# nextpyp/spr_pick

Measured on AMD Instinct MI355X. Metric: train_patches_per_sec, higher is better.
Workload: dtype f32; 1 GPU; BASELINE configs[1]: ssdn --noise_style gaussian --noise_value var, joint mode, 64x64 patches from 4 synthetic 1024x1024 micrographs, batch 32 per GPU, alpha 0.75, tau 0.01, Adam; fp32 MFMA convolutions (Winograd F(2x2,3x3) for the wide 3x3 layers); per_gpu_batch=32, global_batch=32, patch=64, parallelism=single GPU

## Files before the change

include/sprk.h:

```cpp
#ifndef SPRK_H
#define SPRK_H

#include <stddef.h>
#include <stdint.h>

#ifdef __cplusplus
extern "C" {
#endif

#define SPRK_OK 0
#define SPRK_EINVAL (-1)
#define SPRK_EWORKSPACE (-2)
#define SPRK_ELAUNCH (-3)

#define SPRK_ACT_NONE 0
#define SPRK_ACT_LEAKY 1
#define SPRK_ACT_RELU 2

typedef struct sprk_conv_geom {
    int32_t N, C1, C2, Hin, Win, up1;
    int32_t Cout, Hout, Wout;
    int32_t KH, KW, stride, dil, pad_top, pad_left;
    int32_t dtype;
} sprk_conv_geom;
// ... 107 lines not shown
int sprk_act_bwd_partial(const void *gy, const void *y, void *gpre, float *gbias, int act,
                         int N, int C, int H, int W, int up2, long g_image_stride, int io,
                         void *ws, size_t ws_bytes, sprk_reduce_item *item, void *stream);
int sprk_reduce_items(const sprk_reduce_item *items, int n, void *stream);

int sprk_concat_up_bwd(const float *gin, float *ga, float *gb, int N, int C1, int C2, int H, int W,
                       int up1, void *stream);

int sprk_shift_maxpool2_fwd(const void *x, void *y, int NC, int H, int W, int shift, int io, void *stream);
int sprk_shift_maxpool2_bwd(const void *gy, const void *x, void *gx, int NC, int H, int W, int shift, int act,
                            int io, void *stream);
int sprk_rot4_stack_fwd(const float *x, float *y, int B, int C, int P, void *stream);
int sprk_rot4_stack_bwd(const float *gy, float *gx, int B, int C, int P, void *stream);
int sprk_unrot4_shift_concat_fwd(const void *d, void *f, int B, int C, int P, int io, void *stream);
int sprk_unrot4_shift_concat_bwd(const void *gf, void *gd, int B, int C, int P, int io, void *stream);
int sprk_unrot_act_bwd_eligible(int B, int C, int P, int act);
int sprk_conv2d_fwd_unrot_eligible(const sprk_conv_geom *g, const sprk_conv_epilogue *ep);
int sprk_conv2d_fwd_unrot(const float *x, const float *x2, const float *w, float *f, const sprk_conv_geom *g,
                          const sprk_conv_epilogue *ep, void *ws, size_t ws_bytes, void *stream);
int sprk_unrot_act_bwd(const float *gf, const float *f, float *gpre, float *gbias, int act, int B, int C, int P,
                       void *ws, size_t ws_bytes, sprk_reduce_item *item, void *stream);

size_t sprk_bn_ws_bytes(int N, int C, int HW, int groups);
int sprk_bn_train_fwd(const float *x, float *y, const float *gamma, const float *beta,
                      float *running_mean, float *running_var, float *save_mean, float *save_invstd,
                      int N, int C, int HW, int groups, float momentum, float eps, int relu,
                      void *ws, size_t ws_bytes, void *stream);
int sprk_bn_eval_fwd(const float *x, float *y, const float *gamma, const float *beta,
                     const float *running_mean, const float *running_var,
                     int N, int C, int HW, float eps, int relu, void *stream);
int sprk_bn_train_bwd(const float *gy, const float *x, const float *y, const float *gamma,
                      const float *save_mean, const float *save_invstd,
                      float *gx, float *ggamma, float *gbeta,
                      int N, int C, int HW, int groups, int relu, void *ws, size_t ws_bytes, void *stream);

int sprk_reparam_fwd(const float *out_stats, const float *eps, float *z, int B, int HW, void *stream);
int sprk_reparam_bwd(const float *gz, const float *out_stats, const float *eps, float *g_out_stats,
                     int B, int HW, void *stream);
int sprk_sigmoid_clamp_fwd(const float *x, float *p, long n, void *stream);
int sprk_sigmoid_clamp_bwd(const float *gp, const float *x, float *gx, long n, void *stream);
int sprk_crop_add_fwd(const float *y, const float *x, float *out, long NC, int Ho, int Wo, int Hx, int Wx, int off, int stride,
                      void *stream);
int sprk_crop_embed_bwd(const float *g, float *gx, long NC, int Ho, int Wo, int Hx, int Wx, int off, int stride, void *stream);
int sprk_noise_std_fwd(const float *est, float *noise_std, float *z, int B, int HW, void *stream);
int sprk_noise_std_bwd(const float *g, const float *z, float *g_est, int B, int HW, void *stream);
int sprk_joint_loss_fwd(const float *loss_out, const float *pred, const float *p, const float *pf, float *final_loss,
// ... 129 lines not shown
```

spr_pick_amd/_lib.py:

```python
import ctypes
import os

_HERE = os.path.dirname(os.path.abspath(__file__))
LIB_PATH = os.environ.get("SPRK_LIB") or os.path.join(_HERE, "libsprk.so")

ACT_NONE, ACT_LEAKY, ACT_RELU = 0, 1, 2
DT_F32, DT_BF16, DT_F16 = 0, 1, 2
DT_NAIVE = 0x200
DT_WPREP = 0x800
DT_X16, DT_Y16 = 0x8000, 0x10000
DT_PIN = 0x400
DT_FORCE = 0x100
DTYPES = {"f32": DT_F32, "fp32": DT_F32, "bf16": DT_BF16, "f16": DT_F16, "fp16": DT_F16,
          "bf16!": DT_BF16 | DT_FORCE, "f16!": DT_F16 | DT_FORCE}

c_f = ctypes.c_void_p
c_i = ctypes.c_int
c_vp = ctypes.c_void_p
c_sz = ctypes.c_size_t


class ConvGeom(ctypes.Structure):
    _fields_ = [(n, ctypes.c_int32) for n in
                ("N", "C1", "C2", "Hin", "Win", "up1", "Cout", "Hout", "Wout",
# ... 51 lines not shown
    "sprk_conv2d_storage16": (c_i, [ctypes.POINTER(ConvGeom), ctypes.POINTER(ConvEpilogue)]),
    "sprk_conv2d_bwd_weight": (c_i, [c_f, c_f, c_f, c_f, ctypes.POINTER(ConvGeom), c_vp, c_sz, c_vp]),
    "sprk_conv2d_bwd_weight_partial": (c_i, [c_f, c_f, c_f, c_f, ctypes.POINTER(ConvGeom), c_vp, c_sz, ctypes.POINTER(ReduceItem), c_vp]),
    "sprk_act_bwd_partial": (c_i, [c_f, c_f, c_f, c_f, c_i, c_i, c_i, c_i, c_i, c_i, ctypes.c_long, c_i, c_vp, c_sz, ctypes.POINTER(ReduceItem), c_vp]),
    "sprk_reduce_items": (c_i, [ctypes.POINTER(ReduceItem), c_i, c_vp]),
    "sprk_act_bwd_ws_bytes": (c_sz, [c_i, c_i, c_i]),
    "sprk_act_bwd": (c_i, [c_f, c_f, c_f, c_f, c_i, c_i, c_i, c_i, c_i, c_i, ctypes.c_long, c_i, c_vp, c_sz, c_vp]),
    "sprk_concat_up_bwd": (c_i, [c_f, c_f, c_f, c_i, c_i, c_i, c_i, c_i, c_i, c_vp]),
    "sprk_shift_maxpool2_fwd": (c_i, [c_f, c_f, c_i, c_i, c_i, c_i, c_i, c_vp]),
    "sprk_shift_maxpool2_bwd": (c_i, [c_f, c_f, c_f, c_i, c_i, c_i, c_i, c_i, c_i, c_vp]),
    "sprk_rot4_stack_fwd": (c_i, [c_f, c_f, c_i, c_i, c_i, c_vp]),
    "sprk_rot4_stack_bwd": (c_i, [c_f, c_f, c_i, c_i, c_i, c_vp]),
    "sprk_unrot4_shift_concat_fwd": (c_i, [c_f, c_f, c_i, c_i, c_i, c_i, c_vp]),
    "sprk_unrot4_shift_concat_bwd": (c_i, [c_f, c_f, c_i, c_i, c_i, c_i, c_vp]),
    "sprk_unrot_act_bwd_eligible": (c_i, [c_i, c_i, c_i, c_i]),
    "sprk_conv2d_fwd_unrot_eligible": (c_i, [ctypes.POINTER(ConvGeom), ctypes.POINTER(ConvEpilogue)]),
    "sprk_conv2d_bwd_data_mask_fused": (c_i, [ctypes.POINTER(ConvGeom)]),
    "sprk_conv2d_variant": (c_i, [c_i, ctypes.POINTER(ConvGeom), ctypes.POINTER(ConvEpilogue), c_vp, c_vp, c_vp,
                                  ctypes.POINTER(ctypes.c_int32)]),
    "sprk_conv2d_last_variant": (c_i, [c_i, ctypes.POINTER(ctypes.c_int32)]),
    "sprk_conv2d_fwd_unrot": (c_i, [c_f, c_f, c_f, c_f, ctypes.POINTER(ConvGeom), ctypes.POINTER(ConvEpilogue), c_vp, c_sz, c_vp]),
    "sprk_unrot_act_bwd": (c_i, [c_f, c_f, c_f, c_f, c_i, c_i, c_i, c_i, c_vp, c_sz, ctypes.POINTER(ReduceItem), c_vp]),
    "sprk_bn_ws_bytes": (c_sz, [c_i, c_i, c_i, c_i]),
    "sprk_bn_train_fwd": (c_i, [c_f, c_f, c_f, c_f, c_f, c_f, c_f, c_f, c_i, c_i, c_i, c_i, ctypes.c_float, ctypes.c_float, c_i, c_vp, c_sz, c_vp]),
    "sprk_bn_eval_fwd": (c_i, [c_f, c_f, c_f, c_f, c_f, c_f, c_i, c_i, c_i, ctypes.c_float, c_i, c_vp]),
    "sprk_bn_train_bwd": (c_i, [c_f, c_f, c_f, c_f, c_f, c_f, c_f, c_f, c_f, c_i, c_i, c_i, c_i, c_i, c_vp, c_sz, c_vp]),
    "sprk_crop_add_fwd": (c_i, [c_f, c_f, c_f, ctypes.c_long, c_i, c_i, c_i, c_i, c_i, c_i, c_vp]),
    "sprk_crop_embed_bwd": (c_i, [c_f, c_f, ctypes.c_long, c_i, c_i, c_i, c_i, c_i, c_i, c_vp]),
    "sprk_noise_std_fwd": (c_i, [c_f, c_f, c_f, c_i, c_i, c_vp]),
    "sprk_noise_std_bwd": (c_i, [c_f, c_f, c_f, c_i, c_i, c_vp]),
    "sprk_joint_loss_fwd": (c_i, [c_f, c_f, c_f, c_f, c_f, c_f, c_i, c_i, c_i, c_i, ctypes.c_float, ctypes.c_float, c_vp]),
    "sprk_joint_loss_bwd": (c_i, [c_f, c_f, c_f, c_f, c_f, c_f, c_f, c_i, c_i, c_i, c_i, ctypes.c_float, ctypes.c_float, c_vp]),
    "sprk_reparam_fwd": (c_i, [c_f, c_f, c_f, c_i, c_i, c_vp]),
    "sprk_reparam_bwd": (c_i, [c_f, c_f, c_f, c_f, c_i, c_i, c_vp]),
    "sprk_adam_multi": (c_i, [c_vp, c_vp, c_i, c_i, c_f, c_f, c_f, ctypes.c_float, ctypes.c_float, ctypes.c_float, c_vp]),
    "sprk_adam_multi_skip": (c_i, [c_vp, c_vp, c_i, c_i, c_f, c_f, c_f, ctypes.c_float, ctypes.c_float, ctypes.c_float, c_vp, c_vp]),
    "sprk_unscale_check": (c_i, [c_f, ctypes.c_long, c_f, c_vp, c_vp]),
    "sprk_loss_scale_update": (c_i, [c_f, c_f, c_vp, c_vp, c_vp, c_vp, ctypes.c_float, ctypes.c_float, c_i, c_vp]),
    "sprk_pu_loss": (c_i, [c_f, c_f, c_f, c_i, ctypes.c_float, c_f, c_f, c_vp]),
    "sprk_sigmoid_clamp_fwd": (c_i, [c_f, c_f, ctypes.c_long, c_vp]),
    "sprk_sigmoid_clamp_bwd": (c_i, [c_f, c_f, c_f, ctypes.c_long, c_vp]),
    "sprk_ssdn_ws_bytes": (c_sz, [c_i, c_i]),
    "sprk_ssdn_fwd": (c_i, [c_f, c_f, c_f, c_f, c_f, c_f, c_f, c_i, c_i, c_i, c_vp, c_sz, c_vp]),
    "sprk_ssdn_bwd": (c_i, [c_f, c_f, c_f, c_f, c_f, c_f, c_i, c_i, c_i, c_vp, c_sz, c_vp]),
    "sprk_nms2d_ws_bytes": (c_sz, [c_i, c_i, c_i]),
    "sprk_nms2d": (c_i, [c_f, c_i, c_i, c_i, ctypes.c_float, c_f, c_vp, c_vp, c_i, c_i, c_i, c_vp, c_sz, c_vp]),
# ... 79 lines not shown
```

spr_pick_amd/csrc/bn.hip:

```cpp
#include "common.h"

namespace {

constexpr int kBlk = 256;

__device__ __forceinline__ double block_sum(double v, double *red) {
    red[threadIdx.x] = v;
    __syncthreads();
    for (int w = kBlk / 2; w > 0; w >>= 1) {
        if ((int)threadIdx.x < w) red[threadIdx.x] += red[threadIdx.x + w];
        __syncthreads();
    }
    const double r = red[0];
    __syncthreads();
    return r;
}

__device__ __forceinline__ long elem_index(long e, int c, int C, int HW) {
    const long n = e / HW, i = e - n * HW;
    return (n * C + c) * HW + i;
}

template <bool BWD>
__global__ __launch_bounds__(kBlk) void bn_partial_kernel(const float *__restrict__ x, const float *__restrict__ gy,
                                                          const float *__restrict__ y,
                                                          const float *__restrict__ save_mean,
                                                          const float *__restrict__ save_invstd,
                                                          double *__restrict__ partial, int N, int C, int HW, long per,
                                                          int relu) {
    __shared__ double red[kBlk];
    const int c = blockIdx.x, s = blockIdx.y, S = gridDim.y, grp = blockIdx.z;
    const long M = (long)N * HW;
    const long gofs = (long)grp * N * C * HW;
    x += gofs;
    if (BWD) gy += gofs, y = y ? y + gofs : y;
    partial += (long)grp * C * S * 2;
    const long lo = (long)s * per, hi = min(M, lo + per);
    const float mean = BWD ? save_mean[grp * C + c] : 0.f, invstd = BWD ? save_invstd[grp * C + c] : 0.f;
    double a = 0.0, b = 0.0;
    for (long e = lo + threadIdx.x; e < hi; e += kBlk) {
        const long idx = elem_index(e, c, C, HW);
        if (BWD) {
            float g = gy[idx];
            if (relu && !(y[idx] > 0.f)) g = 0.f;
            a += g;
            b += (double)g * (double)((x[idx] - mean) * invstd);
        } else {
            const float v = x[idx];
            a += v;
            b += (double)v * (double)v;
        }
    }
    const double ta = block_sum(a, red), tb = block_sum(b, red);
    if (threadIdx.x == 0) {
        partial[((long)c * S + s) * 2] = ta;
        partial[((long)c * S + s) * 2 + 1] = tb;
    }
}

__global__ __launch_bounds__(kBlk) void bn_train_apply_kernel(const float *__restrict__ x, float *__restrict__ y,
                                                              const float *__restrict__ gamma,
                                                              const float *__restrict__ beta, float *running_mean,
                                                              float *running_var, float *save_mean, float *save_invstd,
                                                              const double *__restrict__ partial, int N, int C, int HW,
                                                              long per, float momentum, float eps, int relu) {
    const int c = blockIdx.x, s = blockIdx.y, S = gridDim.y, grp = blockIdx.z, G = gridDim.z;
    const long M = (long)N * HW;
    auto stats = [&](int gi, double &mean_d, double &var_d) {
        const double *pp = partial + (long)gi * C * S * 2;
        double sa = 0.0, sb = 0.0;
        for (int i = 0; i < S; ++i) {
            sa += pp[((long)c * S + i) * 2];
            sb += pp[((long)c * S + i) * 2 + 1];
        }
        mean_d = sa / (double)M;
        var_d = sb / (double)M - mean_d * mean_d;
        if (var_d < 0.0) var_d = 0.0;
    };
    double mean_d, var_d;
    stats(grp, mean_d, var_d);
    const float mean = (float)mean_d, invstd = (float)(1.0 / sqrt(var_d + (double)eps));
    if (s == 0 && threadIdx.x == 0) {
        save_mean[grp * C + c] = mean;
        save_invstd[grp * C + c] = invstd;
        if (running_mean && grp == 0) {
            float rm = running_mean[c], rv = running_var[c];
            for (int gi = 0; gi < G; ++gi) {
                double m2, v2;
                stats(gi, m2, v2);
                const double unbiased = M > 1 ? v2 * (double)M / (double)(M - 1) : v2;
                rm = (1.f - momentum) * rm + momentum * (float)m2;
                rv = (1.f - momentum) * rv + momentum * (float)unbiased;
            }
            running_mean[c] = rm;
            running_var[c] = rv;
        }
    }
    const long gofs = (long)grp * N * C * HW;
    x += gofs;
    y += gofs;
    const float g = gamma ? gamma[c] : 1.f, b = beta ? beta[c] : 0.f;
    const long lo = (long)s * per, hi = min(M, lo + per);
    for (long e = lo + threadIdx.x; e < hi; e += kBlk) {
        const long idx = elem_index(e, c, C, HW);
        float v = (x[idx] - mean) * invstd * g + b;
        if (relu) v = v > 0.f ? v : 0.f;
        y[idx] = v;
    }
}

__global__ __launch_bounds__(kBlk) void bn_train_bwd_apply_kernel(const float *__restrict__ gy,
                                                                  const float *__restrict__ x,
                                                                  const float *__restrict__ y,
                                                                  const float *__restrict__ gamma,
                                                                  const float *__restrict__ save_mean,
                                                                  const float *__restrict__ save_invstd,
                                                                  float *__restrict__ gx, float *__restrict__ ggamma,
                                                                  float *__restrict__ gbeta,
                                                                  const double *__restrict__ partial, int N, int C,
                                                                  int HW, long per, int relu) {
    const int c = blockIdx.x, s = blockIdx.y, S = gridDim.y, grp = blockIdx.z, G = gridDim.z;
    const long M = (long)N * HW;
    auto sums = [&](int gi, float &sg, float &sgx) {
        const double *pp = partial + (long)gi * C * S * 2;
        double sa = 0.0, sb = 0.0;
        for (int i = 0; i < S; ++i) {
            sa += pp[((long)c * S + i) * 2];
            sb += pp[((long)c * S + i) * 2 + 1];
        }
        sg = (float)sa;
        sgx = (float)sb;
    };
    float sum_g, sum_gx;
    sums(grp, sum_g, sum_gx);
    if (s == 0 && grp == 0 && threadIdx.x == 0) {
        float tg = sum_g, tgx = sum_gx;
        for (int gi = 1; gi < G; ++gi) {
            float a2, b2;
            sums(gi, a2, b2);
            tg += a2;
            tgx += b2;
        }
        if (ggamma) ggamma[c] = tgx;
        if (gbeta) gbeta[c] = tg;
    }
    const long gofs = (long)grp * N * C * HW;
    gy += gofs;
    x += gofs;
    if (y) y += gofs;
    gx += gofs;
    const float mean = save_mean[grp * C + c], invstd = save_invstd[grp * C + c];
    const float k = (gamma ? gamma[c] : 1.f) * invstd, invM = 1.f / (float)M;
    const long lo = (long)s * per, hi = min(M, lo + per);
    for (long e = lo + threadIdx.x; e < hi; e += kBlk) {
        const long idx = elem_index(e, c, C, HW);
        float g = gy[idx];
        if (relu && !(y[idx] > 0.f)) g = 0.f;
        const float xhat = (x[idx] - mean) * invstd;
        gx[idx] = k * (g - sum_g * invM - xhat * sum_gx * invM);
    }
}

__global__ void bn_eval_fwd_kernel(const float *__restrict__ x, float *__restrict__ y, const float *__restrict__ gamma,
                                   const float *__restrict__ beta, const float *__restrict__ rm,
                                   const float *__restrict__ rv, long total, int C, int HW, float eps, int relu) {
    for (long e = (long)blockIdx.x * blockDim.x + threadIdx.x; e < total; e += (long)gridDim.x * blockDim.x) {
        const int c = (int)((e / HW) % C);
        const float invstd = rsqrtf(rv[c] + eps);
        float v = (x[e] - rm[c]) * invstd * (gamma ? gamma[c] : 1.f) + (beta ? beta[c] : 0.f);
        if (relu) v = v > 0.f ? v : 0.f;
        y[e] = v;
    }
}

int slices(int N, int C, int HW) {
    const long M = (long)N * HW;
    long S = 1;
    while ((long)C * S < 1024 && M / (S * 2) >= 2048) S *= 2;
    return (int)S;
}

}

extern "C" {

size_t sprk_bn_ws_bytes(int N, int C, int HW, int groups) {
    if (groups < 1 || N % groups) return 0;
    return (size_t)groups * C * slices(N / groups, C, HW) * 2 * sizeof(double);
}

int sprk_bn_train_fwd(const float *x, float *y, const float *gamma, const float *beta, float *running_mean,
                      float *running_var, float *save_mean, float *save_invstd, int N, int C, int HW, int groups,
                      float momentum, float eps, int relu, void *ws, size_t ws_bytes, void *stream) {
    SPRK_REQUIRE(x && y && save_mean && save_invstd && N > 0 && C > 0 && HW > 0, "bn_train_fwd: bad arguments");
    SPRK_REQUIRE(groups >= 1 && groups <= 64 && N % groups == 0, "bn_train_fwd: the batch does not divide into the groups");
    SPRK_REQUIRE((running_mean == nullptr) == (running_var == nullptr), "bn_train_fwd: running stats mismatch");
    const int Ng = N / groups;
    const int S = slices(Ng, C, HW);
    if (!ws || ws_bytes < (size_t)groups * C * S * 2 * sizeof(double)) {
        sprk::set_error("bn_train_fwd: workspace too small");
        return SPRK_EWORKSPACE;
    }
    const long per = ((long)Ng * HW + S - 1) / S;
    hipStream_t s = (hipStream_t)stream;
    hipLaunchKernelGGL(bn_partial_kernel<false>, dim3(C, S, groups), dim3(kBlk), 0, s, x, (const float *)nullptr,
                       (const float *)nullptr, (const float *)nullptr, (const float *)nullptr, (double *)ws, Ng, C, HW,
                       per, 0);
    if (int rc = sprk::check_launch("bn_partial")) return rc;
    hipLaunchKernelGGL(bn_train_apply_kernel, dim3(C, S, groups), dim3(kBlk), 0, s, x, y, gamma, beta, running_mean,
                       running_var, save_mean, save_invstd, (const double *)ws, Ng, C, HW, per, momentum, eps, relu);
    return sprk::check_launch("bn_train_apply");
}

int sprk_bn_eval_fwd(const float *x, float *y, const float *gamma, const float *beta, const float *running_mean,
                     const float *running_var, int N, int C, int HW, float eps, int relu, void *stream) {
    SPRK_REQUIRE(x && y && running_mean && running_var && N > 0 && C > 0 && HW > 0, "bn_eval_fwd: bad arguments");
    const long total = (long)N * C * HW;
    hipLaunchKernelGGL(bn_eval_fwd_kernel, dim3(sprk::ew_blocks(total)), dim3(256), 0, (hipStream_t)stream, x, y, gamma,
                       beta, running_mean, running_var, total, C, HW, eps, relu);
    return sprk::check_launch("bn_eval_fwd");
}

int sprk_bn_train_bwd(const float *gy, const float *x, const float *y, const float *gamma, const float *save_mean,
                      const float *save_invstd, float *gx, float *ggamma, float *gbeta, int N, int C, int HW, int groups,
                      int relu, void *ws, size_t ws_bytes, void *stream) {
    SPRK_REQUIRE(gy && x && save_mean && save_invstd && gx && N > 0 && C > 0 && HW > 0, "bn_train_bwd: bad arguments");
    SPRK_REQUIRE(groups >= 1 && groups <= 64 && N % groups == 0, "bn_train_bwd: the batch does not divide into the groups");
    SPRK_REQUIRE(!relu || y, "bn_train_bwd: relu needs the saved output");
    const int Ng = N / groups;
    const int S = slices(Ng, C, HW);
    if (!ws || ws_bytes < (size_t)groups * C * S * 2 * sizeof(double)) {
        sprk::set_error("bn_train_bwd: workspace too small");
        return SPRK_EWORKSPACE;
    }
    const long per = ((long)Ng * HW + S - 1) / S;
    hipStream_t s = (hipStream_t)stream;
    hipLaunchKernelGGL(bn_partial_kernel<true>, dim3(C, S, groups), dim3(kBlk), 0, s, x, gy, y, save_mean, save_invstd,
                       (double *)ws, Ng, C, HW, per, relu);
    if (int rc = sprk::check_launch("bn_partial_bwd")) return rc;
    hipLaunchKernelGGL(bn_train_bwd_apply_kernel, dim3(C, S, groups), dim3(kBlk), 0, s, gy, x, y, gamma, save_mean,
                       save_invstd, gx, ggamma, gbeta, (const double *)ws, Ng, C, HW, per, relu);
    return sprk::check_launch("bn_train_bwd_apply");
}

}
```

spr_pick_amd/csrc/conv.hip:

```cpp
#include "common.h"
#include "conv16.h"
#include "gemm1x1.h"
#include "mask1x1.h"
#include "wgrad16.h"
#include "wgrad1x1.h"
#include "wgrad3x3.h"
#include "wino.h"
#include "wprep_dev.h"

#include <cstdlib>

#include "conv_dev.h"
#include "io_dev.h"


namespace {

inline bool naive_of(const sprk_conv_geom *g) { return (g->dtype & SPRK_DT_NAIVE) != 0; }

constexpr int kZeroFloats = 256;
__device__ __attribute__((aligned(64))) float g_zero_block[kZeroFloats];

__device__ __forceinline__ void stage_planes(float *dst, const float *base, long imgStride, long cs, int nch, int N,
                                             int Hin, int Win, int Ws, int up, int vec, const float *zeros,
// ... 712 lines not shown
        for (int ky = 0; ky < g.KH; ++ky) {
            const int ny = iy + g.pad_top - ky * g.dil;
            if (ny < 0 || ny % g.stride) continue;
            const int oy = ny / g.stride;
            if (oy >= g.Hout) continue;
            for (int kx = 0; kx < g.KW; ++kx) {
                const int nx = ix + g.pad_left - kx * g.dil;
                if (nx < 0 || nx % g.stride) continue;
                const int ox = nx / g.stride;
                if (ox >= g.Wout) continue;
                for (int co = 0; co < g.Cout; ++co)
                    s += a.gy[(((long)n * g.Cout + co) * g.Hout + oy) * g.Wout + ox] *
                         a.w[(((long)co * Cin + c) * g.KH + ky) * g.KW + kx];
            }
        }
        a.y[e] = s;
    }
}

constexpr int kStemTW = 32, kStemTH = 8;
constexpr size_t kStemLdsLimit = 64 * 1024;

struct StemPlan {
    int wr, wc, tilesX, tilesY;
    size_t ldsBytes;
};

bool plan_stem_bwd(const sprk_conv_geom *g, StemPlan *p) {
    if (g->stride < 1 || g->dil < 1) return false;
    const long Cin = g->C1 + g->C2;
    p->wr = (kStemTH - 1 + (g->KH - 1) * g->dil) / g->stride + 1;
    p->wc = (kStemTW - 1 + (g->KW - 1) * g->dil) / g->stride + 1;
    p->tilesX = sprk::cdiv(g->Win, kStemTW);
    p->tilesY = sprk::cdiv(g->Hin, kStemTH);
    const long floats = (long)g->Cout * Cin * g->KH * g->KW + (long)g->Cout * p->wr * p->wc;
    p->ldsBytes = (size_t)floats * sizeof(float);
    return p->ldsBytes <= kStemLdsLimit && (long)g->N * p->tilesX * p->tilesY < (1L << 31);
}

__global__ __launch_bounds__(kStemTW * kStemTH) void conv_bwd_data_stem_kernel(const DirectArgs a, int wr, int wc,
                                                                               int tilesX, int tilesY) {
    extern __shared__ __attribute__((aligned(16))) float stem_lds[];
    const sprk_conv_geom &g = a.g;
    const int Cin = g.C1 + g.C2, KHW = g.KH * g.KW;
    const int nW = g.Cout * Cin * KHW;
    float *wl = stem_lds, *gl = stem_lds + nW;
    int bid = blockIdx.x;
    const int tx = bid % tilesX; bid /= tilesX;
    const int ty = bid % tilesY;
    const int n = bid / tilesY;
    const int iy0 = ty * kStemTH, ix0 = tx * kStemTW;
    const int ylo = iy0 + g.pad_top - (g.KH - 1) * g.dil, xlo = ix0 + g.pad_left - (g.KW - 1) * g.dil;
    const int oyLo = ylo <= 0 ? 0 : (ylo + g.stride - 1) / g.stride;
    const int oxLo = xlo <= 0 ? 0 : (xlo + g.stride - 1) / g.stride;
    const int tid = threadIdx.x;
    for (int i = tid; i < nW; i += kStemTW * kStemTH) wl[i] = a.w[i];
    const int win = wr * wc;
    for (int i = tid; i < g.Cout * win; i += kStemTW * kStemTH) {
        const int co = i / win, rem = i - co * win;
        const int r = rem / wc, oy = oyLo + r, ox = oxLo + rem - r * wc;
        gl[i] = (oy < g.Hout && ox < g.Wout) ? a.gy[(((long)n * g.Cout + co) * g.Hout + oy) * g.Wout + ox] : 0.f;
    }
    __syncthreads();
    const int iy = iy0 + tid / kStemTW, ix = ix0 + tid % kStemTW;
    if (iy >= g.Hin || ix >= g.Win) return;
    for (int c = 0; c < Cin; ++c) {
        float s = 0.f;
        for (int ky = 0; ky < g.KH; ++ky) {
            const int ny = iy + g.pad_top - ky * g.dil;
            if (ny < 0 || ny % g.stride) continue;
            const int oy = ny / g.stride;
            if (oy >= g.Hout) continue;
            for (int kx = 0; kx < g.KW; ++kx) {
                const int nx = ix + g.pad_left - kx * g.dil;
                if (nx < 0 || nx % g.stride) continue;
                const int ox = nx / g.stride;
                if (ox >= g.Wout) continue;
                const float *gp = gl + (oy - oyLo) * wc + (ox - oxLo);
                const float *wp = wl + (c * g.KH + ky) * g.KW + kx;
                for (int co = 0; co < g.Cout; ++co) s += gp[co * win] * wp[co * Cin * KHW];
            }
        }
        a.y[(((long)n * Cin + c) * g.Hin + iy) * g.Win + ix] = s;
    }
}

__global__ __launch_bounds__(256) void conv_bwd_weight_direct_kernel(const DirectArgs a) {
    const sprk_conv_geom &g = a.g;
    const int Cin = g.C1 + g.C2;
    const int co = blockIdx.x / Cin, c = blockIdx.x % Cin;
    __shared__ float red[256];
    const long npix = (long)g.N * g.Hout * g.Wout;
    for (int ky = 0; ky < g.KH; ++ky)
        for (int kx = 0; kx < g.KW; ++kx) {
            float s = 0.f;
            for (long p = threadIdx.x; p < npix; p += 256) {
                long t = p;
                const int ox = (int)(t % g.Wout); t /= g.Wout;
                const int oy = (int)(t % g.Hout);
                const int n = (int)(t / g.Hout);
                s += fetch_in(a, n, c, oy * g.stride - g.pad_top + ky * g.dil, ox * g.stride - g.pad_left + kx * g.dil) *
                     a.gy[(((long)n * g.Cout + co) * g.Hout + oy) * g.Wout + ox];
            }
// ... 742 lines not shown
    SPRK_REQUIRE(!unrot || sprk_conv2d_fwd_unrot_eligible(g, ep), "conv2d_fwd_unrot: no kernel with an un-rotated store for this layer");
    SPRK_REQUIRE(x && w && y, "%s: null tensor", who);
    if (bwd) {
        SPRK_REQUIRE(mask_act == SPRK_ACT_NONE || (mask_y && !g->up1), "conv2d_bwd_data: mask needs the saved input, no upsampling");
        if (mask_act == SPRK_ACT_NONE) mask_y = nullptr;
    } else {
        SPRK_REQUIRE(g->C2 == 0 || x2, "conv2d_fwd: C2 > 0 but x2 is null");
        SPRK_REQUIRE(!ep || !ep->scale || ep->shift, "conv2d_fwd: scale without shift");
    }
    hipStream_t s = (hipStream_t)stream;
    auto masked = [&](int rc) { return (rc || !mask_y) ? rc : mask_in_place(y, mask_y, mask_act, g, s); };

    FwdPlan p;
    const FwdVariant v = fwd_route(bwd, g, ep, x, x2, y, mask_y, &p, unrot);
    if (!sprk::wprep_describing()) t_last_fwd[bwd ? 1 : 0] = v;

    if (v.stage == SPRK_STAGE_DIRECT || v.stage == SPRK_STAGE_STEM) {
        if (sprk::wprep_describing()) return SPRK_OK;
        if (bwd) {
            DirectArgs a{nullptr, nullptr, w, x, y, *g, sprk::kNoEpilogue};
            StemPlan sp;
            if (v.stage == SPRK_STAGE_STEM && plan_stem_bwd(g, &sp)) {
                hipLaunchKernelGGL(conv_bwd_data_stem_kernel, dim3(g->N * sp.tilesX * sp.tilesY), dim3(kStemTW * kStemTH),
                                   sp.ldsBytes, s, a, sp.wr, sp.wc, sp.tilesX, sp.tilesY);
                return masked(sprk::check_launch("conv_bwd_data_stem"));
            }
            const long total = (long)g->N * (g->C1 + g->C2) * g->Hin * g->Win;
            hipLaunchKernelGGL(conv_bwd_data_direct_kernel, dim3(sprk::ew_blocks(total)), dim3(256), 0, s, a);
            return masked(sprk::check_launch("conv_bwd_data_direct"));
        }
        DirectArgs a{x, x2, w, nullptr, y, *g, ep ? *ep : sprk::kNoEpilogue};
        const long total = (long)g->N * g->Cout * g->Hout * g->Wout;
        hipLaunchKernelGGL(conv_fwd_direct_kernel, dim3(sprk::ew_blocks(total)), dim3(256), 0, s, a);
        return sprk::check_launch("conv_fwd_direct");
    }
    const sprk::Corr c = bwd ? sprk::Corr(*g) : sprk::Corr(*g, ep);

    if (v.stage == SPRK_STAGE_16BIT) return masked(sprk::conv16_run(c, x, x2, w, y, ws, ws_bytes, s));
    if (int rc = check_storage32(who, c.dtype)) return rc;

    if (v.stage == SPRK_STAGE_WINOGRAD) {
        if (int rc = sprk::check_ws(who, ws, ws_bytes, sprk::wino_ws_bytes(c))) return rc;
        if (int rc = sprk::wino_conv(c, v.wino, x, x2, w, y, (float *)ws, mask_y, mask_act, s)) return rc;
        return sprk::check_launch(bwd ? "wino_conv(bwd_data)" : "wino_conv");
    }
    SPRK_REQUIRE(!unrot, "conv2d_fwd_unrot: the call left the Winograd stage");

// ... 366 lines not shown
```

Before: 2082 patches/s.

## Fuse small BatchNorm stats and apply into one LDS kernel; vectorize stem backward

Adds a single-launch BatchNorm forward and backward for small per-channel sizes. One 1024-thread block per channel stages the channel in LDS, reduces the statistics and applies the result, replacing the separate partial and apply kernels. The existing BN kernels switch to an incremental index walker instead of per-element division, and use a cheaper tree reduction. The stem backward-data conv now stores weights and gradients channel-innermost with padding, uses float4 dot products, and skips kernel taps that cannot be live under the stride. The cost is more code paths, different FP summation order, and low parallelism when there are few channels.

```diff
diff --git a/include/sprk.h b/include/sprk.h
--- a/include/sprk.h
+++ b/include/sprk.h
@@ -153,6 +153,9 @@
                        void *ws, size_t ws_bytes, sprk_reduce_item *item, void *stream);
 
 size_t sprk_bn_ws_bytes(int N, int C, int HW, int groups);
+int sprk_bn_plan(int N, int C, int HW, int groups, int *S, int *fused);
+void sprk_bn_fused_enable(int on);
+long sprk_bn_fused_launch_count(void);
 int sprk_bn_train_fwd(const float *x, float *y, const float *gamma, const float *beta,
                       float *running_mean, float *running_var, float *save_mean, float *save_invstd,
                       int N, int C, int HW, int groups, float momentum, float eps, int relu,
diff --git a/scratch/bn_stem_trace_summary.py b/scratch/bn_stem_trace_summary.py
--- /dev/null
+++ b/scratch/bn_stem_trace_summary.py
@@ -0,0 +1,20 @@
+import csv, glob, os, re, sys
+from collections import defaultdict
+d, steps = sys.argv[1], int(sys.argv[2])
+pat = re.compile(r"bn_|conv_bwd_data_stem|gemm1x1_kernel<2|wino_conv_kernel<6, 0, 1|unrot_act_bwd64")
+def short(n):
+    n = re.sub(r"\(anonymous namespace\)::", "", n); n = re.sub(r"^void ", "", n)
+    return n.split("(")[0][:60]
+tot, cnt, allt = defaultdict(float), defaultdict(int), 0.0
+for f in glob.glob(os.path.join(d, "**", "*kernel_trace.csv"), recursive=True):
+    for r in csv.DictReader(open(f)):
+        us = (int(r["End_Timestamp"]) - int(r["Start_Timestamp"])) / 1e3
+        allt += us
+        k = short(r["Kernel_Name"])
+        if pat.search(k):
+            tot[k] += us; cnt[k] += 1
+for k in sorted(tot):
+    print("%-45s launches/step %6.2f  us/step %8.1f" % (k, cnt[k] / steps, tot[k] / steps))
+bn = [k for k in tot if k.startswith("bn_") and "eval" not in k]
+print("%-45s launches/step %6.2f  us/step %8.1f" % ("all BatchNorm (training)", sum(cnt[k] for k in bn) / steps, sum(tot[k] for k in bn) / steps))
+print("%-45s us/step %8.1f" % ("all kernels", allt / steps))
diff --git a/scratch/bn_sweep.py b/scratch/bn_sweep.py
--- /dev/null
+++ b/scratch/bn_sweep.py
@@ -0,0 +1,40 @@
+import os
+import sys
+
+sys.path.insert(0, os.path.dirname(os.path.dirname(os.path.abspath(__file__))))
+import torch
+from spr_pick_amd import _lib, torch_ops
+L = _lib.lib(); S = torch.ops.sprk; d = torch.device("cuda:0")
+SH = [(1, 4096), (32, 841), (32, 729), (32, 529), (32, 441), (64, 81), (64, 49), (64, 9), (128, 1)]
+def bench(N, C, HW, on):
+    L.sprk_bn_fused_enable(on)
+    x = torch.randn(N, C, HW, 1, device=d); gy = torch.randn_like(x)
+    ga, be = torch.rand(C, device=d) + .5, torch.randn(C, device=d); rm, rv = torch.zeros(C, device=d), torch.ones(C, device=d)
+    gg, gb = torch.empty_like(ga), torch.empty_like(ga)
+    def pair():
+        y, m, i = S.bn_train_fwd(x, ga, be, rm, rv, 0.1, 1e-5, True, 2)
+        return S.bn_train_bwd(gy, x, y, ga, m, i, True, 2, gg, gb)
+    def fwd():
+        return S.bn_train_fwd(x, ga, be, rm, rv, 0.1, 1e-5, True, 2)
+    out = []
+    for fn in (fwd, pair):
+        side = torch.cuda.Stream(); side.wait_stream(torch.cuda.current_stream())
+        with torch.cuda.stream(side):
+            fn()
+        torch.cuda.current_stream().wait_stream(side); torch.cuda.synchronize()
+        g = torch.cuda.CUDAGraph()
+        with torch.cuda.graph(g):
+            for _ in range(20): fn()
+        g.replay(); torch.cuda.synchronize()
+        ts = []
+        for _ in range(20):
+            a, b = torch.cuda.Event(enable_timing=True), torch.cuda.Event(enable_timing=True)
+            a.record(); g.replay(); b.record(); torch.cuda.synchronize(); ts.append(a.elapsed_time(b) * 1e3 / 20)
+        ts.sort(); out.append(ts[len(ts) // 2])
+    return out[0], out[1] - out[0]
+for batch in (32, 16):
+    for C, HW in SH:
+        r = {on: bench(2 * batch, C, HW, on) for on in (0, 1, 0, 1)}
+        print("batch %2d C %3d HW %4d M/group %6d | two kernels fwd %6.1f bwd %6.1f us | fused switch on fwd %6.1f bwd %6.1f us"
+              % (batch, C, HW, batch * HW, r[0][0], r[0][1], r[1][0], r[1][1]), flush=True)
+L.sprk_bn_fused_enable(1)
diff --git a/spr_pick_amd/_lib.py b/spr_pick_amd/_lib.py
--- a/spr_pick_amd/_lib.py
+++ b/spr_pick_amd/_lib.py
@@ -97,6 +97,9 @@
     "sprk_conv2d_fwd_unrot": (c_i, [c_f, c_f, c_f, c_f, ctypes.POINTER(ConvGeom), ctypes.POINTER(ConvEpilogue), c_vp, c_sz, c_vp]),
     "sprk_unrot_act_bwd": (c_i, [c_f, c_f, c_f, c_f, c_i, c_i, c_i, c_i, c_vp, c_sz, ctypes.POINTER(ReduceItem), c_vp]),
     "sprk_bn_ws_bytes": (c_sz, [c_i, c_i, c_i, c_i]),
+    "sprk_bn_plan": (c_i, [c_i, c_i, c_i, c_i, ctypes.POINTER(ctypes.c_int), ctypes.POINTER(ctypes.c_int)]),
+    "sprk_bn_fused_enable": (None, [c_i]),
+    "sprk_bn_fused_launch_count": (ctypes.c_long, []),
     "sprk_bn_train_fwd": (c_i, [c_f, c_f, c_f, c_f, c_f, c_f, c_f, c_f, c_i, c_i, c_i, c_i, ctypes.c_float, ctypes.c_float, c_i, c_vp, c_sz, c_vp]),
     "sprk_bn_eval_fwd": (c_i, [c_f, c_f, c_f, c_f, c_f, c_f, c_i, c_i, c_i, ctypes.c_float, c_i, c_vp]),
     "sprk_bn_train_bwd": (c_i, [c_f, c_f, c_f, c_f, c_f, c_f, c_f, c_f, c_f, c_i, c_i, c_i, c_i, c_i, c_vp, c_sz, c_vp]),
diff --git a/spr_pick_amd/csrc/bn.hip b/spr_pick_amd/csrc/bn.hip
--- a/spr_pick_amd/csrc/bn.hip
+++ b/spr_pick_amd/csrc/bn.hip
@@ -1,24 +1,132 @@
 #include "common.h"
 
+namespace sprk {
+std::atomic<long> g_bn_fused_launches{0};
+std::atomic<int> g_bn_fused_on{1};
+}
+
 namespace {
 
 constexpr int kBlk = 256;
-
-__device__ __forceinline__ double block_sum(double v, double *red) {
-    red[threadIdx.x] = v;
+constexpr int kFusedThreads = 1024;
+constexpr int kFusedQ = kFusedThreads / kBlk;
+constexpr int kRed = 2 * 192;
+constexpr long kFusedMaxElems = 4096;
+constexpr int kFusedMinChannels = 16;
+constexpr long kFusedSmallElems = 8192;
+
+struct Walk {
+    long idx, didx, wrap;
+    int i, di, HW;
+    __device__ __forceinline__ Walk(long e, int c, int C, int HW_, int step) : HW(HW_) {
+        const long n = e / HW;
+        i = (int)(e - n * HW);
+        idx = (n * C + c) * HW + i;
+        const int dn = step / HW;
+        di = step - dn * HW;
+        didx = (long)dn * C * HW + di;
+        wrap = (long)(C - 1) * HW;
+    }
+    __device__ __forceinline__ void next() {
+        i += di;
+        idx += didx;
+        if (i >= HW) {
+            i -= HW;
+            idx += wrap;
+        }
+    }
+};
+
+__device__ __forceinline__ void acc_fwd(double &a, double &b, float v) {
+#pragma clang fp contract(off)
+    a += (double)v;
+    b = fma((double)v, (double)v, b);
+}
+
+__device__ __forceinline__ float xhat_of(float x, float mean, float invstd) {
+#pragma clang fp contract(off)
+    return (x - mean) * invstd;
+}
+
+__device__ __forceinline__ void acc_bwd(double &a, double &b, float g, float xhat) {
+#pragma clang fp contract(off)
+    a += (double)g;
+    b = fma((double)g, (double)xhat, b);
+}
+
+__device__ __forceinline__ float masked_grad(float g, const float *__restrict__ y, long idx, int relu) {
+    return (relu && !(y[idx] > 0.f)) ? 0.f : g;
+}
+
+__device__ __forceinline__ void combine(const double *pp, int S, double &sa, double &sb) {
+    sa = 0.0, sb = 0.0;
+    for (int i = 0; i < S; ++i) {
+        sa += pp[2 * i];
+        sb += pp[2 * i + 1];
+    }
+}
+
+__device__ __forceinline__ void batch_stats(double sa, double sb, long M, double &mean_d, double &var_d) {
+#pragma clang fp contract(off)
+    mean_d = sa / (double)M;
+    var_d = fma(-mean_d, mean_d, sb / (double)M);
+    if (var_d < 0.0) var_d = 0.0;
+}
+
+__device__ __forceinline__ float invstd_of(double var_d, float eps) {
+#pragma clang fp contract(off)
+    return (float)(1.0 / sqrt(var_d + (double)eps));
+}
+
+__device__ __forceinline__ void running_update(float &rm, float &rv, double mean_d, double var_d, long M, float momentum) {
+#pragma clang fp contract(off)
+    const double unbiased = M > 1 ? var_d * (double)M / (double)(M - 1) : var_d;
+    rm = (1.f - momentum) * rm + momentum * (float)mean_d;
+    rv = (1.f - momentum) * rv + momentum * (float)unbiased;
+}
+
+__device__ __forceinline__ float fwd_elem(float x, float mean, float invstd, float g, float b, int relu) {
+#pragma clang fp contract(off)
+    float v = fmaf(g, (x - mean) * invstd, b);
+    if (relu) v = v > 0.f ? v : 0.f;
+    return v;
+}
+
+__device__ __forceinline__ float bwd_elem(float g, float xhat, float k, float mg, float sum_gx, float invM) {
+#pragma clang fp contract(off)
+    return k * fmaf(-invM, xhat * sum_gx, g - mg);
+}
+
+__device__ __forceinline__ void bwd_consts(float gamma, float invstd, float sum_g, long M, float &k, float &invM, float &mg) {
+#pragma clang fp contract(off)
+    k = gamma * invstd;
+    invM = 1.f / (float)M;
+    mg = sum_g * invM;
+}
+
+__device__ __forceinline__ void tree_sum2(double &a, double &b, double *red, int t) {
+    if (t >= 128) {
+        red[t - 128] = a;
+        red[192 + t - 128] = b;
+    }
     __syncthreads();
-    for (int w = kBlk / 2; w > 0; w >>= 1) {
-        if ((int)threadIdx.x < w) red[threadIdx.x] += red[threadIdx.x + w];
-        __syncthreads();
-    }
-    const double r = red[0];
+    if (t < 128) {
+        a += red[t];
+        b += red[192 + t];
+        if (t >= 64) {
+            red[128 + t - 64] = a;
+            red[192 + 128 + t - 64] = b;
+        }
+    }
     __syncthreads();
-    return r;
-}
-
-__device__ __forceinline__ long elem_index(long e, int c, int C, int HW) {
-    const long n = e / HW, i = e - n * HW;
-    return (n * C + c) * HW + i;
+    if (t < 64) {
+        a += red[128 + t];
+        b += red[192 + 128 + t];
+        for (int w = 32; w > 0; w >>= 1) {
+            a += __shfl_down(a, w);
+            b += __shfl_down(b, w);
+        }
+    }
 }
 
 template <bool BWD>
@@ -28,7 +136,7 @@
                                                           const float *__restrict__ save_invstd,
                                                           double *__restrict__ partial, int N, int C, int HW, long per,
                                                           int relu) {
-    __shared__ double red[kBlk];
+    __shared__ double red[kRed];
     const int c = blockIdx.x, s = blockIdx.y, S = gridDim.y, grp = blockIdx.z;
     const long M = (long)N * HW;
     const long gofs = (long)grp * N * C * HW;
@@ -38,23 +146,20 @@
     const long lo = (long)s * per, hi = min(M, lo + per);
     const float mean = BWD ? save_mean[grp * C + c] : 0.f, invstd = BWD ? save_invstd[grp * C + c] : 0.f;
     double a = 0.0, b = 0.0;
-    for (long e = lo + threadIdx.x; e < hi; e += kBlk) {
-        const long idx = elem_index(e, c, C, HW);
-        if (BWD) {
-            float g = gy[idx];
-            if (relu && !(y[idx] > 0.f)) g = 0.f;
-            a += g;
-            b += (double)g * (double)((x[idx] - mean) * invstd);
-        } else {
-            const float v = x[idx];
-            a += v;
-            b += (double)v * (double)v;
-        }
-    }
-    const double ta = block_sum(a, red), tb = block_sum(b, red);
+    long e = lo + threadIdx.x;
+    if (e < hi) {
+        Walk w(e, c, C, HW, kBlk);
+        for (; e < hi; e += kBlk, w.next()) {
+            if (BWD)
+                acc_bwd(a, b, masked_grad(gy[w.idx], y, w.idx, relu), xhat_of(x[w.idx], mean, invstd));
+            else
+                acc_fwd(a, b, x[w.idx]);
+        }
+    }
+    tree_sum2(a, b, red, threadIdx.x);
     if (threadIdx.x == 0) {
-        partial[((long)c * S + s) * 2] = ta;
-        partial[((long)c * S + s) * 2 + 1] = tb;
+        partial[((long)c * S + s) * 2] = a;
+        partial[((long)c * S + s) * 2 + 1] = b;
     }
 }
 
@@ -67,19 +172,13 @@
     const int c = blockIdx.x, s = blockIdx.y, S = gridDim.y, grp = blockIdx.z, G = gridDim.z;
     const long M = (long)N * HW;
     auto stats = [&](int gi, double &mean_d, double &var_d) {
-        const double *pp = partial + (long)gi * C * S * 2;
-        double sa = 0.0, sb = 0.0;
-        for (int i = 0; i < S; ++i) {
-            sa += pp[((long)c * S + i) * 2];
-            sb += pp[((long)c * S + i) * 2 + 1];
-        }
-        mean_d = sa / (double)M;
-        var_d = sb / (double)M - mean_d * mean_d;
-        if (var_d < 0.0) var_d = 0.0;
+        double sa, sb;
+        combine(partial + ((long)gi * C + c) * S * 2, S, sa, sb);
+        batch_stats(sa, sb, M, mean_d, var_d);
     };
     double mean_d, var_d;
     stats(grp, mean_d, var_d);
-    const float mean = (float)mean_d, invstd = (float)(1.0 / sqrt(var_d + (double)eps));
+    const float mean = (float)mean_d, invstd = invstd_of(var_d, eps);
     if (s == 0 && threadIdx.x == 0) {
         save_mean[grp * C + c] = mean;
         save_invstd[grp * C + c] = invstd;
@@ -88,9 +187,7 @@
             for (int gi = 0; gi < G; ++gi) {
                 double m2, v2;
                 stats(gi, m2, v2);
-                const double unbiased = M > 1 ? v2 * (double)M / (double)(M - 1) : v2;
-                rm = (1.f - momentum) * rm + momentum * (float)m2;
-                rv = (1.f - momentum) * rv + momentum * (float)unbiased;
+                running_update(rm, rv, m2, v2, M, momentum);
             }
             running_mean[c] = rm;
             running_var[c] = rv;
@@ -101,12 +198,10 @@
     y += gofs;
     const float g = gamma ? gamma[c] : 1.f, b = beta ? beta[c] : 0.f;
     const long lo = (long)s * per, hi = min(M, lo + per);
-    for (long e = lo + threadIdx.x; e < hi; e += kBlk) {
-        const long idx = elem_index(e, c, C, HW);
-        float v = (x[idx] - mean) * invstd * g + b;
-        if (relu) v = v > 0.f ? v : 0.f;
-        y[idx] = v;
-    }
+    long e = lo + threadIdx.x;
+    if (e >= hi) return;
+    Walk w(e, c, C, HW, kBlk);
+    for (; e < hi; e += kBlk, w.next()) y[w.idx] = fwd_elem(x[w.idx], mean, invstd, g, b, relu);
 }
 
 __global__ __launch_bounds__(kBlk) void bn_train_bwd_apply_kernel(const float *__restrict__ gy,
@@ -122,12 +217,8 @@
     const int c = blockIdx.x, s = blockIdx.y, S = gridDim.y, grp = blockIdx.z, G = gridDim.z;
     const long M = (long)N * HW;
     auto sums = [&](int gi, float &sg, float &sgx) {
-        const double *pp = partial + (long)gi * C * S * 2;
-        double sa = 0.0, sb = 0.0;
-        for (int i = 0; i < S; ++i) {
-            sa += pp[((long)c * S + i) * 2];
-            sb += pp[((long)c * S + i) * 2 + 1];
-        }
+        double sa, sb;
+        combine(partial + ((long)gi * C + c) * S * 2, S, sa, sb);
         sg = (float)sa;
         sgx = (float)sb;
     };
@@ -150,14 +241,133 @@
     if (y) y += gofs;
     gx += gofs;
     const float mean = save_mean[grp * C + c], invstd = save_invstd[grp * C + c];
-    const float k = (gamma ? gamma[c] : 1.f) * invstd, invM = 1.f / (float)M;
+    float k, invM, mg;
+    bwd_consts(gamma ? gamma[c] : 1.f, invstd, sum_g, M, k, invM, mg);
     const long lo = (long)s * per, hi = min(M, lo + per);
-    for (long e = lo + threadIdx.x; e < hi; e += kBlk) {
-        const long idx = elem_index(e, c, C, HW);
-        float g = gy[idx];
-        if (relu && !(y[idx] > 0.f)) g = 0.f;
-        const float xhat = (x[idx] - mean) * invstd;
-        gx[idx] = k * (g - sum_g * invM - xhat * sum_gx * invM);
+    long e = lo + threadIdx.x;
+    if (e >= hi) return;
+    Walk w(e, c, C, HW, kBlk);
+    for (; e < hi; e += kBlk, w.next())
+        gx[w.idx] = bwd_elem(masked_grad(gy[w.idx], y, w.idx, relu), xhat_of(x[w.idx], mean, invstd), k, mg, sum_gx, invM);
+}
+
+constexpr size_t fused_lds_bytes(long M, int S) {
+    return (size_t)(kFusedQ * kRed + 2 * S) * sizeof(double) + (size_t)M * sizeof(float);
+}
+
+__global__ __launch_bounds__(kFusedThreads) void bn_fused_fwd_kernel(const float *__restrict__ x, float *__restrict__ y,
+                                                                     const float *__restrict__ gamma,
+                                                                     const float *__restrict__ beta, float *running_mean,
+                                                                     float *running_var, float *save_mean,
+                                                                     float *save_invstd, int N, int C, int HW, int G, int S,
+                                                                     int per, float momentum, float eps, int relu) {
+    extern __shared__ __attribute__((aligned(16))) unsigned char bn_lds[];
+    double *red = reinterpret_cast<double *>(bn_lds);
+    double *psum = red + kFusedQ * kRed;
+    float *buf = reinterpret_cast<float *>(psum + 2 * S);
+    const int c = blockIdx.x, tid = threadIdx.x, q = tid / kBlk, t = tid % kBlk;
+    const int M = N * HW;
+    const float g = gamma ? gamma[c] : 1.f, b = beta ? beta[c] : 0.f;
+    float rm = 0.f, rv = 0.f;
+    if (tid == 0 && running_mean) rm = running_mean[c], rv = running_var[c];
+    for (int grp = 0; grp < G; ++grp) {
+        const long gofs = (long)grp * N * C * HW;
+        const float *xg = x + gofs;
+        float *yg = y + gofs;
+        if (tid < M) {
+            Walk w(tid, c, C, HW, kFusedThreads);
+            for (int e = tid; e < M; e += kFusedThreads, w.next()) buf[e] = xg[w.idx];
+        }
+        __syncthreads();
+        for (int s0 = 0; s0 < S; s0 += kFusedQ) {
+            const int s = s0 + q;
+            double a = 0.0, bb = 0.0;
+            if (s < S) {
+                const int lo = s * per, hi = min(M, lo + per);
+                for (int e = lo + t; e < hi; e += kBlk) acc_fwd(a, bb, buf[e]);
+            }
+            tree_sum2(a, bb, red + q * kRed, t);
+            if (s < S && t == 0) psum[2 * s] = a, psum[2 * s + 1] = bb;
+        }
+        __syncthreads();
+        double sa, sb, mean_d, var_d;
+        combine(psum, S, sa, sb);
+        batch_stats(sa, sb, M, mean_d, var_d);
+        const float mean = (float)mean_d, invstd = invstd_of(var_d, eps);
+        if (tid == 0) {
+            save_mean[grp * C + c] = mean;
+            save_invstd[grp * C + c] = invstd;
+            if (running_mean) running_update(rm, rv, mean_d, var_d, M, momentum);
+        }
+        if (tid < M) {
+            Walk w(tid, c, C, HW, kFusedThreads);
+            for (int e = tid; e < M; e += kFusedThreads, w.next()) yg[w.idx] = fwd_elem(buf[e], mean, invstd, g, b, relu);
+        }
+        __syncthreads();
+    }
+    if (tid == 0 && running_mean) running_mean[c] = rm, running_var[c] = rv;
+}
+
+__global__ __launch_bounds__(kFusedThreads) void bn_fused_bwd_kernel(const float *__restrict__ gy, const float *__restrict__ x,
+                                                                     const float *__restrict__ y,
+                                                                     const float *__restrict__ gamma,
+                                                                     const float *__restrict__ save_mean,
+                                                                     const float *__restrict__ save_invstd,
+                                                                     float *__restrict__ gx, float *__restrict__ ggamma,
+                                                                     float *__restrict__ gbeta, int N, int C, int HW, int G,
+                                                                     int S, int per, int relu) {
+    extern __shared__ __attribute__((aligned(16))) unsigned char bn_lds[];
+    double *red = reinterpret_cast<double *>(bn_lds);
+    double *psum = red + kFusedQ * kRed;
+    float *buf = reinterpret_cast<float *>(psum + 2 * S);
+    const int c = blockIdx.x, tid = threadIdx.x, q = tid / kBlk, t = tid % kBlk;
+    const int M = N * HW;
+    const float gam = gamma ? gamma[c] : 1.f;
+    float tg = 0.f, tgx = 0.f;
+    for (int grp = 0; grp < G; ++grp) {
+        const long gofs = (long)grp * N * C * HW;
+        const float *gyg = gy + gofs, *xg = x + gofs, *yg = y ? y + gofs : y;
+        float *gxg = gx + gofs;
+        const float mean = save_mean[grp * C + c], invstd = save_invstd[grp * C + c];
+        if (tid < M) {
+            Walk w(tid, c, C, HW, kFusedThreads);
+            for (int e = tid; e < M; e += kFusedThreads, w.next()) buf[e] = masked_grad(gyg[w.idx], yg, w.idx, relu);
+        }
+        __syncthreads();
+        for (int s0 = 0; s0 < S; s0 += kFusedQ) {
+            const int s = s0 + q;
+            double a = 0.0, bb = 0.0;
+            if (s < S) {
+                const int lo = s * per, hi = min(M, lo + per);
+                int e = lo + t;
+                if (e < hi) {
+                    Walk w(e, c, C, HW, kBlk);
+                    for (; e < hi; e += kBlk, w.next()) acc_bwd(a, bb, buf[e], xhat_of(xg[w.idx], mean, invstd));
+                }
+            }
+            tree_sum2(a, bb, red + q * kRed, t);
+            if (s < S && t == 0) psum[2 * s] = a, psum[2 * s + 1] = bb;
+        }
+        __syncthreads();
+        double sa, sb;
+        combine(psum, S, sa, sb);
+        const float sum_g = (float)sa, sum_gx = (float)sb;
+        if (tid == 0) {
+            tg = grp ? tg + sum_g : sum_g;
+            tgx = grp ? tgx + sum_gx : sum_gx;
+        }
+        float k, invM, mg;
+        bwd_consts(gam, invstd, sum_g, M, k, invM, mg);
+        if (tid < M) {
+            Walk w(tid, c, C, HW, kFusedThreads);
+            for (int e = tid; e < M; e += kFusedThreads, w.next())
+                gxg[w.idx] = bwd_elem(buf[e], xhat_of(xg[w.idx], mean, invstd), k, mg, sum_gx, invM);
+        }
+        __syncthreads();
+    }
+    if (tid == 0) {
+        if (ggamma) ggamma[c] = tgx;
+        if (gbeta) gbeta[c] = tg;
     }
 }
 
@@ -180,9 +390,39 @@
     return (int)S;
 }
 
+struct BnPlan {
+    int S;
+    long per;
+    bool fused;
+    size_t ldsBytes;
+};
+
+BnPlan plan_bn(int Ng, int C, int HW, int groups) {
+    BnPlan p;
+    const long M = (long)Ng * HW;
+    p.S = slices(Ng, C, HW);
+    p.per = (M + p.S - 1) / p.S;
+    p.fused = sprk::g_bn_fused_on.load(std::memory_order_relaxed) && M <= kFusedMaxElems &&
+              (C >= kFusedMinChannels || (long)groups * M <= kFusedSmallElems);
+    p.ldsBytes = p.fused ? fused_lds_bytes(M, p.S) : 0;
+    return p;
+}
+
 }
 
 extern "C" {
+
+void sprk_bn_fused_enable(int on) { sprk::g_bn_fused_on.store(on ? 1 : 0); }
+long sprk_bn_fused_launch_count(void) { return sprk::g_bn_fused_launches.load(); }
+
+int sprk_bn_plan(int N, int C, int HW, int groups, int *S, int *fused) {
+    SPRK_REQUIRE(N > 0 && C > 0 && HW > 0, "bn_plan: bad arguments");
+    SPRK_REQUIRE(groups >= 1 && groups <= 64 && N % groups == 0, "bn_plan: the batch does not divide into the groups");
+    const BnPlan p = plan_bn(N / groups, C, HW, groups);
+    if (S) *S = p.S;
+    if (fused) *fused = p.fused ? 1 : 0;
+    return SPRK_OK;
+}
 
 size_t sprk_bn_ws_bytes(int N, int C, int HW, int groups) {
     if (groups < 1 || N % groups) return 0;
@@ -196,19 +436,28 @@
     SPRK_REQUIRE(groups >= 1 && groups <= 64 && N % groups == 0, "bn_train_fwd: the batch does not divide into the groups");
     SPRK_REQUIRE((running_mean == nullptr) == (running_var == nullptr), "bn_train_fwd: running stats mismatch");
     const int Ng = N / groups;
-    const int S = slices(Ng, C, HW);
+    const BnPlan p = plan_bn(Ng, C, HW, groups);
+    const int S = p.S;
     if (!ws || ws_bytes < (size_t)groups * C * S * 2 * sizeof(double)) {
         sprk::set_error("bn_train_fwd: workspace too small");
         return SPRK_EWORKSPACE;
     }
-    const long per = ((long)Ng * HW + S - 1) / S;
     hipStream_t s = (hipStream_t)stream;
+    if (p.fused) {
+        if (int rc = sprk::lds_optin(bn_fused_fwd_kernel, p.ldsBytes, "bn_fused_fwd")) return rc;
+        hipLaunchKernelGGL(bn_fused_fwd_kernel, dim3(C), dim3(kFusedThreads), p.ldsBytes, s, x, y, gamma, beta,
+                           running_mean, running_var, save_mean, save_invstd, Ng, C, HW, groups, S, (int)p.per, momentum,
+                           eps, relu);
+        if (int rc = sprk::check_launch("bn_fused_fwd")) return rc;
+        sprk::g_bn_fused_launches.fetch_add(1, std::memory_order_relaxed);
+        return SPRK_OK;
+    }
     hipLaunchKernelGGL(bn_partial_kernel<false>, dim3(C, S, groups), dim3(kBlk), 0, s, x, (const float *)nullptr,
                        (const float *)nullptr, (const float *)nullptr, (const float *)nullptr, (double *)ws, Ng, C, HW,
-                       per, 0);
+                       p.per, 0);
     if (int rc = sprk::check_launch("bn_partial")) return rc;
     hipLaunchKernelGGL(bn_train_apply_kernel, dim3(C, S, groups), dim3(kBlk), 0, s, x, y, gamma, beta, running_mean,
-                       running_var, save_mean, save_invstd, (const double *)ws, Ng, C, HW, per, momentum, eps, relu);
+                       running_var, save_mean, save_invstd, (const double *)ws, Ng, C, HW, p.per, momentum, eps, relu);
     return sprk::check_launch("bn_train_apply");
 }
 
@@ -228,18 +477,26 @@
     SPRK_REQUIRE(groups >= 1 && groups <= 64 && N % groups == 0, "bn_train_bwd: the batch does not divide into the groups");
     SPRK_REQUIRE(!relu || y, "bn_train_bwd: relu needs the saved output");
     const int Ng = N / groups;
-    const int S = slices(Ng, C, HW);
+    const BnPlan p = plan_bn(Ng, C, HW, groups);
+    const int S = p.S;
     if (!ws || ws_bytes < (size_t)groups * C * S * 2 * sizeof(double)) {
         sprk::set_error("bn_train_bwd: workspace too small");
         return SPRK_EWORKSPACE;
     }
-    const long per = ((long)Ng * HW + S - 1) / S;
     hipStream_t s = (hipStream_t)stream;
+    if (p.fused) {
+        if (int rc = sprk::lds_optin(bn_fused_bwd_kernel, p.ldsBytes, "bn_fused_bwd")) return rc;
+        hipLaunchKernelGGL(bn_fused_bwd_kernel, dim3(C), dim3(kFusedThreads), p.ldsBytes, s, gy, x, y, gamma, save_mean,
+                           save_invstd, gx, ggamma, gbeta, Ng, C, HW, groups, S, (int)p.per, relu);
+        if (int rc = sprk::check_launch("bn_fused_bwd")) return rc;
+        sprk::g_bn_fused_launches.fetch_add(1, std::memory_order_relaxed);
+        return SPRK_OK;
+    }
     hipLaunchKernelGGL(bn_partial_kernel<true>, dim3(C, S, groups), dim3(kBlk), 0, s, x, gy, y, save_mean, save_invstd,
-                       (double *)ws, Ng, C, HW, per, relu);
+                       (double *)ws, Ng, C, HW, p.per, relu);
     if (int rc = sprk::check_launch("bn_partial_bwd")) return rc;
     hipLaunchKernelGGL(bn_train_bwd_apply_kernel, dim3(C, S, groups), dim3(kBlk), 0, s, gy, x, y, gamma, save_mean,
-                       save_invstd, gx, ggamma, gbeta, (const double *)ws, Ng, C, HW, per, relu);
+                       save_invstd, gx, ggamma, gbeta, (const double *)ws, Ng, C, HW, p.per, relu);
     return sprk::check_launch("bn_train_bwd_apply");
 }
 
diff --git a/spr_pick_amd/csrc/conv.hip b/spr_pick_amd/csrc/conv.hip
--- a/spr_pick_amd/csrc/conv.hip
+++ b/spr_pick_amd/csrc/conv.hip
@@ -758,7 +758,7 @@
 constexpr size_t kStemLdsLimit = 64 * 1024;
 
 struct StemPlan {
-    int wr, wc, tilesX, tilesY;
+    int wr, wc, tilesX, tilesY, ldc, kstep, ostep;
     size_t ldsBytes;
 };
 
@@ -769,18 +769,29 @@
     p->wc = (kStemTW - 1 + (g->KW - 1) * g->dil) / g->stride + 1;
     p->tilesX = sprk::cdiv(g->Win, kStemTW);
     p->tilesY = sprk::cdiv(g->Hin, kStemTH);
-    const long floats = (long)g->Cout * Cin * g->KH * g->KW + (long)g->Cout * p->wr * p->wc;
+    p->ldc = sprk::cdiv(g->Cout, 4) * 4 + 4;
+    int gcd = g->stride;
+    for (int b = g->dil; b;) {
+        const int r = gcd % b;
+        gcd = b;
+        b = r;
+    }
+    p->kstep = g->stride / gcd;
+    p->ostep = g->dil / gcd;
+    const long floats = (Cin * g->KH * g->KW + (long)p->wr * p->wc) * p->ldc;
     p->ldsBytes = (size_t)floats * sizeof(float);
     return p->ldsBytes <= kStemLdsLimit && (long)g->N * p->tilesX * p->tilesY < (1L << 31);
 }
 
 __global__ __launch_bounds__(kStemTW * kStemTH) void conv_bwd_data_stem_kernel(const DirectArgs a, int wr, int wc,
-                                                                               int tilesX, int tilesY) {
+                                                                               int tilesX, int tilesY, int ldc, int kstep,
+                                                                               int ostep) {
     extern __shared__ __attribute__((aligned(16))) float stem_lds[];
+    constexpr int T = kStemTW * kStemTH;
     const sprk_conv_geom &g = a.g;
-    const int Cin = g.C1 + g.C2, KHW = g.KH * g.KW;
-    const int nW = g.Cout * Cin * KHW;
-    float *wl = stem_lds, *gl = stem_lds + nW;
+    const int Cin = g.C1 + g.C2, KHW = g.KH * g.KW, CK = Cin * KHW;
+    const int nW = g.Cout * CK;
+    float *wl = stem_lds, *gl = stem_lds + CK * ldc;
     int bid = blockIdx.x;
     const int tx = bid % tilesX; bid /= tilesX;
     const int ty = bid % tilesY;
@@ -790,31 +801,61 @@
     const int oyLo = ylo <= 0 ? 0 : (ylo + g.stride - 1) / g.stride;
     const int oxLo = xlo <= 0 ? 0 : (xlo + g.stride - 1) / g.stride;
     const int tid = threadIdx.x;
-    for (int i = tid; i < nW; i += kStemTW * kStemTH) wl[i] = a.w[i];
+    if (tid < nW) {
+        int co = tid / CK, r = tid - co * CK;
+        const int dco = T / CK, dr = T - dco * CK;
+        for (int i = tid; i < nW; i += T) {
+            wl[r * ldc + co] = a.w[i];
+            co += dco, r += dr;
+            if (r >= CK) r -= CK, ++co;
+        }
+    }
     const int win = wr * wc;
-    for (int i = tid; i < g.Cout * win; i += kStemTW * kStemTH) {
-        const int co = i / win, rem = i - co * win;
-        const int r = rem / wc, oy = oyLo + r, ox = oxLo + rem - r * wc;
-        gl[i] = (oy < g.Hout && ox < g.Wout) ? a.gy[(((long)n * g.Cout + co) * g.Hout + oy) * g.Wout + ox] : 0.f;
+    if (tid < g.Cout * win) {
+        int co = tid / win, r = (tid - co * win) / wc, col = tid - co * win - r * wc;
+        const int dco = T / win, dr = (T - dco * win) / wc, dcol = T - dco * win - dr * wc;
+        for (int i = tid; i < g.Cout * win; i += T) {
+            const int oy = oyLo + r, ox = oxLo + col;
+            gl[(r * wc + col) * ldc + co] =
+                (oy < g.Hout && ox < g.Wout) ? a.gy[(((long)n * g.Cout + co) * g.Hout + oy) * g.Wout + ox] : 0.f;
+            co += dco, r += dr, col += dcol;
+            if (col >= wc) col -= wc, ++r;
+            if (r >= wr) r -= wr, ++co;
+        }
     }
     __syncthreads();
     const int iy = iy0 + tid / kStemTW, ix = ix0 + tid % kStemTW;
     if (iy >= g.Hin || ix >= g.Win) return;
+    auto first_live = [&](int p, int K, int &k0, int &o0) {
+        k0 = K, o0 = -1;
+        for (int k = 0; k < kstep && k < K; ++k)
+            if ((p - k * g.dil) % g.stride == 0) {
+                k0 = k, o0 = (p - k * g.dil) / g.stride;
+                break;
+            }
+    };
+    int ky0, oy0, kx0, ox0;
+    first_live(iy + g.pad_top, g.KH, ky0, oy0);
+    first_live(ix + g.pad_left, g.KW, kx0, ox0);
+    const int Cout4 = g.Cout & ~3;
     for (int c = 0; c < Cin; ++c) {
         float s = 0.f;
-        for (int ky = 0; ky < g.KH; ++ky) {
-            const int ny = iy + g.pad_top - ky * g.dil;
-            if (ny < 0 || ny % g.stride) continue;
-            const int oy = ny / g.stride;
+        for (int ky = ky0, oy = oy0; ky < g.KH && oy >= 0; ky += kstep, oy -= ostep) {
             if (oy >= g.Hout) continue;
-            for (int kx = 0; kx < g.KW; ++kx) {
-                const int nx = ix + g.pad_left - kx * g.dil;
-                if (nx < 0 || nx % g.stride) continue;
-                const int ox = nx / g.stride;
+            for (int kx = kx0, ox = ox0; kx < g.KW && ox >= 0; kx += kstep, ox -= ostep) {
                 if (ox >= g.Wout) continue;
-                const float *gp = gl + (oy - oyLo) * wc + (ox - oxLo);
-                const float *wp = wl + (c * g.KH + ky) * g.KW + kx;
-                for (int co = 0; co < g.Cout; ++co) s += gp[co * win] * wp[co * Cin * KHW];
+                const float *gp = gl + ((oy - oyLo) * wc + (ox - oxLo)) * ldc;
+                const float *wp = wl + ((c * g.KH + ky) * g.KW + kx) * ldc;
+#pragma unroll 4
+                for (int co = 0; co < Cout4; co += 4) {
+                    const float4 gv = *reinterpret_cast<const float4 *>(gp + co);
+                    const float4 wv = *reinterpret_cast<const float4 *>(wp + co);
+                    s = fmaf(gv.x, wv.x, s);
+                    s = fmaf(gv.y, wv.y, s);
+                    s = fmaf(gv.z, wv.z, s);
+                    s = fmaf(gv.w, wv.w, s);
+                }
+                for (int co = Cout4; co < g.Cout; ++co) s += gp[co] * wp[co];
             }
         }
         a.y[(((long)n * Cin + c) * g.Hin + iy) * g.Win + ix] = s;
@@ -1603,7 +1644,7 @@
             StemPlan sp;
             if (v.stage == SPRK_STAGE_STEM && plan_stem_bwd(g, &sp)) {
                 hipLaunchKernelGGL(conv_bwd_data_stem_kernel, dim3(g->N * sp.tilesX * sp.tilesY), dim3(kStemTW * kStemTH),
-                                   sp.ldsBytes, s, a, sp.wr, sp.wc, sp.tilesX, sp.tilesY);
+                                   sp.ldsBytes, s, a, sp.wr, sp.wc, sp.tilesX, sp.tilesY, sp.ldc, sp.kstep, sp.ostep);
                 return masked(sprk::check_launch("conv_bwd_data_stem"));
             }
             const long total = (long)g->N * (g->C1 + g->C2) * g->Hin * g->Win;
```

Result: no change. 2101 patches/s, median of 6 (+0.9%).
